# tkkiran/Robust-Conditional-GAN

Hardware: AMD Instinct MI355X
Metric: images/sec G+D train step (CIFAR-10 RCGAN bs=64) (higher is better)
Workload: dtype bf16

## Files before the change

### include/rcgan_hip.h

```cpp
#ifndef RCGAN_HIP_H
#define RCGAN_HIP_H

#include <stddef.h>
#include <stdint.h>

#ifdef __cplusplus
extern "C" {
#endif

#define RCGAN_OK 0
#define RCGAN_EINVALID_ARG (-1)
#define RCGAN_EUNSUPPORTED_SHAPE (-2)
#define RCGAN_EWORKSPACE_TOO_SMALL (-3)
#define RCGAN_EHIP (-4)
#define RCGAN_ERCCL (-5)

#define RCGAN_F32 0
#define RCGAN_BF16 1
#define RCGAN_F16 2

#define RCGAN_ACT_NONE 0
#define RCGAN_ACT_RELU 1
#define RCGAN_ACT_LRELU 2
#define RCGAN_ACT_TANH 3
// ... 285 lines not shown
int rcgan_poly3_rowsum(rcgan_ctx* ctx, int nq, int nr, int d, int n_seg, const float* q, const int32_t* q_off, const float* r,
                       const int32_t* r_off, double gamma, double coef0, int exclude_same_row, double* rowsum);

int rcgan_adam_tf(rcgan_ctx* ctx, size_t count, float* w, const float* g, float* m, float* v,
                  const float* hyper, float beta1, float beta2, float eps, float clip, float grad_scale);
int rcgan_adam_tf_host(rcgan_ctx* ctx, size_t count, float* w, const float* g, float* m, float* v,
                       float lr, float t, float beta1, float beta2, float eps, float clip, float grad_scale);
int rcgan_fill_f32(rcgan_ctx* ctx, size_t count, float* p, float value);
int rcgan_copy_words(rcgan_ctx* ctx, size_t count, const void* src, void* dst);

int rcgan_conv_stats_ok(const rcgan_conv_desc* d);
size_t rcgan_conv_stats_bytes(const rcgan_conv_desc* d);
int rcgan_conv2d_fwd_stats(rcgan_ctx* ctx, const rcgan_conv_desc* d, const void* x, const void* prepared, const float* bias,
                           const void* residual, void* y, float* tile_sums);
int rcgan_bn_stats_from_tiles(rcgan_ctx* ctx, const rcgan_conv_desc* d, int nseg, float eps, const float* tile_sums, float* mean, float* rstd);
int rcgan_bn_apply_segments(rcgan_ctx* ctx, int nseg, int n_per_seg, int rows_per_sample, int c, int n_labels, int dtype, const void* x,
                            const int32_t* labels, const float* gamma, const float* beta, const float* mean, const float* rstd, int act,
                            void* y, void* ws, size_t ws_bytes);

int rcgan_set_grad_scale(rcgan_ctx* ctx, float host_scale, const float* dev_scale);

#define RCGAN_F32_PRECISION_HIGHEST 0
#define RCGAN_F32_PRECISION_HIGH 1
int rcgan_set_f32_matmul_precision(rcgan_ctx* ctx, int precision);
int rcgan_grad_finite_check(rcgan_ctx* ctx, size_t count, const float* g, float* ls_state);
int rcgan_adam_tf_dyn(rcgan_ctx* ctx, size_t count, float* w, const float* g, float* m, float* v, float lr, const float* t_dev,
                      float beta1, float beta2, float eps, float clip, float grad_scale, const float* ls_state);
int rcgan_loss_scale_update(rcgan_ctx* ctx, float* ls_state, float* t_dev0, float* t_dev1, float growth_interval, float min_scale,
                            float max_scale);

// ... 26 lines not shown
```

### robust-conditional-gan_amd/_lib.py

```python
import ctypes as C
import os

_HERE = os.path.dirname(os.path.abspath(__file__))
LIB_PATH = os.environ.get("RCGAN_LIB_PATH") or os.path.join(_HERE, "librcgan_hip.so")
LIB_PATH_F16 = os.environ.get("RCGAN_LIB_PATH_F16") or os.path.join(_HERE, "librcgan_hip_f16.so")

F32, BF16, F16 = 0, 1, 2
ACT_NONE, ACT_RELU, ACT_LRELU, ACT_TANH, ACT_SIGMOID = 0, 1, 2, 3, 4
CONV_IN_UPSAMPLE2X, CONV_IN_RELU, CONV_ACCUMULATE, CONV_FORCE_DIRECT, CONV_OUT_MEANPOOL2, CONV_RESID_UPSAMPLE2X = 1, 2, 4, 8, 16, 32
LOSS_HINGE_REAL, LOSS_HINGE_FAKE, LOSS_NEG_MEAN, LOSS_CE_ONES, LOSS_CE_ZEROS = 0, 1, 2, 3, 4
QUERY_TR_READ = 0
AUG_COLOR, AUG_TRANSLATION, AUG_CUTOUT = 1, 2, 4
AUG_POLICIES = {"color": AUG_COLOR, "translation": AUG_TRANSLATION, "cutout": AUG_CUTOUT}
F32_PRECISION_HIGHEST, F32_PRECISION_HIGH = 0, 1
F32_PRECISIONS = {"highest": F32_PRECISION_HIGHEST, "high": F32_PRECISION_HIGH}

RCGAN_EHIP, RCGAN_ERCCL = -4, -5
EINVALID_ARG, EUNSUPPORTED_SHAPE, EWORKSPACE_TOO_SMALL = -1, -2, -3
ERRORS = {-1: "RCGAN_EINVALID_ARG", -2: "RCGAN_EUNSUPPORTED_SHAPE", -3: "RCGAN_EWORKSPACE_TOO_SMALL",
          -4: "RCGAN_EHIP", -5: "RCGAN_ERCCL"}


def source_hash():
    import glob
# ... 195 lines not shown
    "rcgan_class_moments_bytes": (SZ, [I, I]),
    "rcgan_class_moments_accum": (I, [P, I, I, I, P, P, P]),
    "rcgan_knn_radius": (I, [P, I, I, I, I, P, P, P]),
    "rcgan_ball_query": (I, [P, I, I, I, I, P, P, P, P, P, P, P]),
    "rcgan_poly3_rowsum": (I, [P, I, I, I, I, P, P, P, P, C.c_double, C.c_double, I, P]),
    "rcgan_sgd_momentum": (I, [P, SZ, SZ, P, P, P, P, F, F, I, F]),
    "rcgan_augment_cifar": (I, [P, I, I, P, P, P, P, I, I, P, P]),
    "rcgan_adam_tf": (I, [P, SZ, P, P, P, P, P, F, F, F, F, F]),
    "rcgan_adam_tf_host": (I, [P, SZ, P, P, P, P, F, F, F, F, F, F, F]),
    "rcgan_fill_f32": (I, [P, SZ, P, F]),
    "rcgan_copy_words": (I, [P, SZ, P, P]),
    "rcgan_conv_stats_ok": (I, [DP]),
    "rcgan_conv_stats_bytes": (SZ, [DP]),
    "rcgan_conv2d_fwd_stats": (I, [P, DP, P, P, P, P, P, P]),
    "rcgan_bn_stats_from_tiles": (I, [P, DP, I, F, P, P, P]),
    "rcgan_bn_apply_segments": (I, [P, I, I, I, I, I, I, P, P, P, P, P, P, I, P, P, SZ]),
    "rcgan_comm_unique_id": (I, [P]),
    "rcgan_comm_init": (I, [P, P, I, I]),
    "rcgan_comm_init_stub": (I, [P, I]),
    "rcgan_comm_destroy": (I, [P]),
    "rcgan_comm_world": (I, [P]),
    "rcgan_allreduce_sum": (I, [P, P, SZ]),
    "rcgan_allreduce_sum_buckets": (I, [P, I, P, P]),
    "rcgan_allreduce_sum_async": (I, [P, P, SZ]),
    "rcgan_allreduce_join": (I, [P]),
    "rcgan_comm_count": (I, [P, P]),
    "rcgan_allreduce_bf16_scratch_bytes": (SZ, [I, P]),
    "rcgan_allreduce_sum_bf16_buckets": (I, [P, I, P, P, P, SZ]),
    "rcgan_comm_stub_model": (I, [P, C.c_double, C.c_double]),
    "rcgan_comm_load_error": (C.c_char_p, []),
# ... 33 lines not shown
```

### robust-conditional-gan_amd/csrc/api.hip

```cpp
#include "conv_wgrad.h"
#include "small_gemm.h"
#include "step_inputs.h"
#include "conv_image.h"


size_t direct_wgrad_ws_bytes(const rcgan_conv_desc* d);
template <typename T> int direct_fwd(rcgan_ctx*, const rcgan_conv_desc*, const T*, const float*, const float*, const float*, T*, int n_cols = 0);
template <typename T> int direct_dgrad(rcgan_ctx*, const rcgan_conv_desc*, const T*, const float*, const float*, const float*, const T*, T*, int);
template <typename T> int direct_wgrad(rcgan_ctx*, const rcgan_conv_desc*, const T*, const T*, float*, float*, int, void*, size_t);
template <typename T> int direct_wgrad_cols(rcgan_ctx*, const rcgan_conv_desc*, const T*, const T*, int, const float*, float*, int, void*, size_t);
size_t direct_wgrad_cols_ws_bytes(const rcgan_conv_desc* d, int c1);
template <typename T> int colsum_launch(rcgan_ctx*, const T*, long, int, float*, int, float*);
template <typename T> int linear_fwd(rcgan_ctx*, long, long, long, const T*, const float*, const float*, const float*, T*);
template <typename T> int linear_dgrad(rcgan_ctx*, long, long, long, const T*, const float*, const float*, T*, int);
template <typename T> int linear_wgrad(rcgan_ctx*, long, long, long, const T*, const T*, float*, float*, int, void*, size_t);
size_t linear_wgrad_ws_bytes(long m, long k, long n);
template <typename T> int sumpool2_masked_launch(rcgan_ctx*, int, int, int, int, const T*, const T*, T*, int);
int small_fwd_kind(const rcgan_conv_desc* d);
int small_dgrad_kind(const rcgan_conv_desc* d);
int small_wgrad_kind(const rcgan_conv_desc* d);
size_t small_wgrad_ws_bytes(const rcgan_conv_desc* d);
template <typename T> int small_fwd(rcgan_ctx*, const rcgan_conv_desc*, int, const T*, const float*, const float*, T*);
template <typename T> int small_dgrad(rcgan_ctx*, const rcgan_conv_desc*, int, const T*, const float*, T*, int);
template <typename T> int small_wgrad(rcgan_ctx*, const rcgan_conv_desc*, int, const T*, const T*, float*, float*, int, void*, size_t);
// ... 566 lines not shown
      a.PT = d->kh - 1 - a.PT; a.PL = d->kw - 1 - a.PL;
      if (up) a.accumulate = 0;
    }
  }
  return RCGAN_OK;
}

int rcgan_conv2d_fwd(rcgan_ctx* ctx, const rcgan_conv_desc* d, const void* x, const void* prepared, const float* bias, void* y) {
  return rcgan_conv2d_fwd_residual(ctx, d, x, prepared, bias, nullptr, y);
}

int rcgan_conv_stats_ok(const rcgan_conv_desc* d) {
  if (!d || !mfma_eligible(d) || d->stride != 1 || d->cout != 256) return 0;
  if (d->flags & (RCGAN_CONV_OUT_MEANPOOL2 | RCGAN_CONV_ACCUMULATE | RCGAN_CONV_IN_RELU | RCGAN_CONV_FORCE_DIRECT)) return 0;
  if (((long)d->n * d->h * d->w) % 256 != 0) return 0;
  if ((d->flags & RCGAN_CONV_RESID_UPSAMPLE2X) && !rcgan_conv_resid_up_ok(d)) return 0;
  MfmaConvArgs a;
  if (mfma_conv_pose(nullptr, d, CONV_FWD, nullptr, nullptr, nullptr, false, nullptr, &a)) return 0;
  if (a.up && !(mfma_phase_filters(d) && mfma_conv8_phase_form(a))) return 0;
  return mfma_conv_is_p8(a) ? 1 : 0;
}

size_t rcgan_conv_stats_bytes(const rcgan_conv_desc* d) {
  return d ? (size_t)((long)d->n * d->h * d->w / 256) * d->cout * 2 * sizeof(float) : 0;
}

int rcgan_conv2d_fwd_stats(rcgan_ctx* ctx, const rcgan_conv_desc* d, const void* x, const void* prepared, const float* bias,
                           const void* residual, void* y, float* tile_sums) {
  int rc = check_desc(ctx, d);
  if (rc) return rc;
// ... 55 lines not shown
  int rc = check_desc(ctx, d);
  if (rc) return rc;
  RC_REQUIRE(ctx, x && prepared && y && mean && rstd && gamma && beta, "null argument");
  RC_REQUIRE(ctx, segments >= 1 && d->n % segments == 0, "segments must divide the batch");
  if (!rcgan_conv_bn_in_ok(d)) RC_FAIL(ctx, RCGAN_EUNSUPPORTED_SHAPE, "no kernel applies a batch norm to this convolution's staged input (rcgan_conv_bn_in_ok)");
  if (residual == nullptr && img_fwd_bn_ok(d)) return img_fwd_bn(ctx, d, x, prepared, bias, y, mean, rstd, gamma, beta, labels, segments, act);
  RC_REQUIRE(ctx, mfma_bn_in_route(d), "residual form needs a halo-patch kernel");
  MfmaConvArgs a;
  rc = mfma_conv_pose(ctx, d, CONV_FWD, x, prepared, bias, residual != nullptr, y, &a);
  if (rc) return rc;
  rc = ensure_selftest(ctx);
  if (rc) return rc;
  a.resid = (const bf16_t*)residual;
  a.bn_mean = mean; a.bn_rstd = rstd; a.bn_gamma = gamma; a.bn_beta = beta; a.bn_labels = labels;
  a.bn_seg_samples = d->n / segments; a.bn_act = act;
  return mfma_conv_launch(ctx, a);
}

int rcgan_conv2d_fwd_residual(rcgan_ctx* ctx, const rcgan_conv_desc* d, const void* x, const void* prepared, const float* bias,
                              const void* residual, void* y) {
  int rc = check_desc(ctx, d);
  if (rc) return rc;
  if (residual != nullptr && !mfma_eligible(d)) {
    RC_REQUIRE(ctx, !(d->flags & RCGAN_CONV_RESID_UPSAMPLE2X), "half-resolution residual not available for this convolution (rcgan_conv_resid_up_ok)");
    RC_REQUIRE(ctx, residual != y, "residual must not alias the output");
    rc = rcgan_conv2d_fwd_residual(ctx, d, x, prepared, bias, nullptr, y);
    if (rc) return rc;
    int oh, ow, p;
    same_pad(d->h, d->kh, d->stride, &oh, &p);
    same_pad(d->w, d->kw, d->stride, &ow, &p);
// ... 230 lines not shown
```

### robust-conditional-gan_amd/csrc/bn.hip

```cpp
#include "common.h"
#include "conv_mfma.h"
#include "bn_plan.h"

template <typename T, int MODE>
__global__ __launch_bounds__(256) void bn_partial_kernel(long rows, int c, long rows_per_group, const T* x, const T* y,
                                                         const T* dy, const float* mean, const float* rstd, int act,
                                                         float* partial) {
  __shared__ float red[2][4][64];
  const int col = blockIdx.x * 64 + (threadIdx.x & 63);
  const int rl = threadIdx.x >> 6;
  const long rb = (long)blockIdx.y * rows_per_group;
  long re = rb + rows_per_group;
  if (re > rows) re = rows;
  float s1 = 0.f, s2 = 0.f;
  if (col < c) {
    float mu = 0.f, rs = 1.f;
    if (MODE == 1) { mu = mean[col]; rs = rstd[col]; }
    for (long r = rb + rl; r < re; r += 4) {
      const long off = r * c + col;
      if (MODE == 0) {
        float v = Elem<T>::ld(x + off);
        s1 += v; s2 += v * v;
      } else {
        float g = Elem<T>::ld(dy + off);
// ... 786 lines not shown
    float o[8];
#pragma unroll
    for (int j = 0; j < 8; ++j) o[j] = rs[j] * gm[j] * gv[j] + p[j] * xv[j] + q[j];
    if (accumulate_dx) {
      float d[8];
      ld8(dx + off, d);
#pragma unroll
      for (int j = 0; j < 8; ++j) o[j] += d[j];
    }
    st8(dx + off, o);
  }
}

__global__ __launch_bounds__(256) void bn_tile_stats_finish_kernel(const float* __restrict__ part, int c, int tps, int ngroups, long group_stride,
                                                                   double inv_count, float eps, float* mean, float* rstd) {
  __shared__ double red[2][16][16];
  const int cl = threadIdx.x & 15, sub = threadIdx.x >> 4, ch = blockIdx.x * 16 + cl, sg = blockIdx.y;
  double s1 = 0.0, s2 = 0.0;
  for (int g = 0; g < ngroups; ++g) {
    const long t0 = (long)g * group_stride + (long)sg * tps;
    for (int tb = sub; tb < tps; tb += 16 * 8) {
      float2 v[8];
#pragma unroll
      for (int q = 0; q < 8; ++q) {
        const int t = tb + q * 16;
        v[q] = t < tps ? *(const float2*)(part + ((t0 + t) * c + ch) * 2) : make_float2(0.f, 0.f);
      }
#pragma unroll
      for (int q = 0; q < 8; ++q) { s1 += (double)v[q].x; s2 += (double)v[q].y; }
    }
  }
  red[0][sub][cl] = s1; red[1][sub][cl] = s2;
  __syncthreads();
  if (sub == 0) {
    double a1 = 0.0, a2 = 0.0;
#pragma unroll
    for (int q = 0; q < 16; ++q) { a1 += red[0][q][cl]; a2 += red[1][q][cl]; }
    const double mu = a1 * inv_count;
    double var = a2 * inv_count - mu * mu;
    if (var < 0.0) var = 0.0;
    mean[(long)sg * c + ch] = (float)mu;
    rstd[(long)sg * c + ch] = (float)(1.0 / sqrt(var + (double)eps));
  }
}

int bn_tile_stats_finish_launch(rcgan_ctx* ctx, const float* part, int c, int nseg, int tiles_per_seg, int ngroups, long group_stride,
                                double count, float eps, float* mean, float* rstd) {
  RC_REQUIRE(ctx, c % 16 == 0 && tiles_per_seg >= 1, "bad tile statistics layout");
  hipLaunchKernelGGL(bn_tile_stats_finish_kernel, dim3(c / 16, nseg), dim3(256), 0, ctx->stream, part, c, tiles_per_seg, ngroups, group_stride,
                     1.0 / count, eps, mean, rstd);
  RC_LAUNCH_CHECK(ctx);
  return RCGAN_OK;
}


template <typename T>
__global__ __launch_bounds__(256) void bn_sample_partial_kernel(int rows_per_sample, int c, const T* x, const T* y, const T* dy,
// ... 399 lines not shown
```

### robust-conditional-gan_amd/csrc/conv_mfma.hip

```cpp
#include <vector>
#include "conv_mfma.h"
#include "small_gemm.h"
#include "step_inputs.h"
#include "mfma_util.h"

#define LDS_PITCH 72

template <int BM, int BN>
__global__ __launch_bounds__(256) void conv_mfma_kernel(MfmaConvArgs a) {
  extern __shared__ __attribute__((aligned(16))) unsigned char smem[];
  bf16_t* As = (bf16_t*)smem;
  bf16_t* Bs = As + 2 * BM * LDS_PITCH;
  constexpr int AR = BM / 32, BR = BN / 32;
  constexpr int TM = BM / 2, TN = BN / 2;
  constexpr int NI = TN / 16, NJ = TM / 16;

  const int tid = threadIdx.x, lane = tid & 63, wave = tid >> 6;
  const int wm = wave & 1, wn = wave >> 1;
  const long m0 = (long)blockIdx.x * BM;
  const int co0 = blockIdx.y * BN;
  const int chunk = tid & 7, lrow = tid >> 3;
  const int K = a.KH * a.KW * a.Cin;
  const int KT = K / 64;
  const int Hs = a.up ? (a.H >> 1) : a.H, Ws = a.up ? (a.W >> 1) : a.W;
// ... 941 lines not shown
static ConvRoute mfma_conv_route(const MfmaConvArgs& a) {
  static const int p8_min = env_int("RCGAN_P8_MINBLK", 200);
  static const int p8n_min = env_int("RCGAN_P8N_MINBLK", 190);
  static const int ks2_max = env_int("RCGAN_KS2_MAXBLK", 576);
  static const int halo = env_int("RCGAN_P8_HALO", 1), halo_n = env_int("RCGAN_P8N_HALO", 1);
  static const int t128_min = env_int("RCGAN_T128_MINBLK", 384);
  static const int t256_min = env_int("RCGAN_T256_MINBLK", 1 << 30);
  if (a.phase == MFMA_FORM_PHASE || a.phase == MFMA_FORM_GATHER) {
    const bool whole = a.phase == MFMA_FORM_PHASE ? ((a.M >> 2) % 256 == 0) : (a.M % 256 == 0);
    const long b8 = (a.M / 256) * (a.Cout / 256), b8n = (a.M / 256) * (a.Cout / 128);
    if (a.phase == MFMA_FORM_GATHER) {
      const int gather_min = env_int("RCGAN_H8N_GATHER_MINBLK", 190);
      if (halo_n && whole && a.Cout % 128 == 0 && b8n >= gather_min && mfma_conv8n_halo_takes(a)) return CR_H8N;
    }
    if (whole && a.Cout % 256 == 0 && b8 >= p8_min && 4 * b8 >= 3 * (long)cdiv(b8, 256) * 256)
      return (halo && !a.stats && mfma_conv8_halo_takes(a)) ? CR_H8 : CR_P8;
    if (whole && a.Cout % 128 == 0 && b8n >= p8n_min)
      return (a.phase == MFMA_FORM_PHASE && halo_n && mfma_conv8n_halo_takes(a)) ? CR_H8N : CR_P8N;
    return (a.M / 64) * (a.Cout / 64) <= ks2_max ? CR_PHASE_KS2 : CR_PHASE;
  }
  MfmaConvArgs b = a;
  b.phase = mfma_conv8_phase_form(a) ? MFMA_FORM_PHASE : MFMA_FORM_PLAIN;
  const bool off32 = (long)a.N * a.H * a.W * a.Cin < (1L << 32);
  const long b8 = (long)cdiv(a.M, 256) * (a.Cout / 256), b8n = (long)cdiv(a.M, 256) * (a.Cout / 128);
  const bool fit8 = 4 * b8 >= 3 * (long)cdiv(b8, 256) * 256;
  if (a.Cout % 256 == 0 && a.zero != nullptr && off32 && b8 >= p8_min && fit8) return (halo && !a.stats && mfma_conv8_halo_takes(b)) ? CR_H8 : CR_P8;
  if (a.Cout % 128 == 0 && a.zero != nullptr && b8n >= p8n_min) return (halo_n && mfma_conv8n_halo_takes(b)) ? CR_H8N : CR_P8N;
  if (a.Cout % 256 == 0 && b8 >= t256_min && a.zero != nullptr) return CR_T256;
  if (a.Cout % 128 == 0 && b8n >= t256_min && a.zero != nullptr) return CR_T256N;
  if (a.Cout % 128 == 0 && (long)cdiv(a.M, 128) * (a.Cout / 128) >= t128_min) return CR_T128;
  return CR_64;
}

bool mfma_conv_is_p8(const MfmaConvArgs& a) {
  if (a.phase != MFMA_FORM_PLAIN || a.Cin % 64 || a.Cout % 64) return false;
  const ConvRoute r = mfma_conv_route(a);
  return r == CR_H8 || r == CR_P8;
}

int mfma_conv_bn_route(const MfmaConvArgs& a) {
  if (a.phase != MFMA_FORM_PLAIN || a.Cin % 64 || a.Cout % 64 || a.zero == nullptr || a.stats || a.relu_in || a.Cin > 1024) return 0;
  const ConvRoute r = mfma_conv_route(a);
  return r == CR_H8 ? 1 : r == CR_H8N ? 2 : 0;
}

int mfma_conv_launch(rcgan_ctx* ctx, const MfmaConvArgs& a_in) {
  MfmaConvArgs a = a_in;
  a.stamps = (unsigned long long*)ctx->dbg_stamps;
  if (a.Cin % 64 || a.Cout % 64) RC_FAIL(ctx, RCGAN_EUNSUPPORTED_SHAPE, "channels %d -> %d", a.Cin, a.Cout);
  const ConvRoute r = mfma_conv_route(a);
  if (a.bn_mean && !(a.phase == MFMA_FORM_PLAIN && !a.stats && !a.relu_in && a.Cin <= 1024 && a.zero != nullptr && (r == CR_H8 || r == CR_H8N)))
    RC_FAIL(ctx, RCGAN_EUNSUPPORTED_SHAPE, "batch norm on the staged input needs a halo-patch kernel (rcgan_conv_bn_in_ok)");
  if (a.stats && !(a.phase == MFMA_FORM_PLAIN && a.zero != nullptr && (r == CR_H8 || r == CR_P8)))
    RC_FAIL(ctx, RCGAN_EUNSUPPORTED_SHAPE, "tile statistics need the 256 x 256 kernel (rcgan_conv_stats_ok)");
  switch (r) {
    case CR_H8: case CR_P8: return mfma_conv8_launch(ctx, a, true, r == CR_H8);
    case CR_H8N: case CR_P8N: return mfma_conv8_launch(ctx, a, false, r == CR_H8N);
    case CR_PHASE_KS2: return a.phase == MFMA_FORM_PHASE ? launch_conv_glds_phase<64, 64, 2, 2, 1>(ctx, a) : launch_conv_glds_phase<64, 64, 2, 2, 2>(ctx, a);
    case CR_PHASE: return a.phase == MFMA_FORM_PHASE ? launch_conv_glds_phase<64, 64, 2, 1, 1>(ctx, a) : launch_conv_glds_phase<64, 64, 2, 1, 2>(ctx, a);
    case CR_T256: return launch_conv_glds<256, 256, 2>(ctx, a);
    case CR_T256N: return launch_conv_glds<256, 128, 2>(ctx, a);
    case CR_T128: return launch_conv_mfma<128, 128>(ctx, a);
    default: return launch_conv_mfma<64, 64>(ctx, a);
  }
}

// ... 60 lines not shown
```

### robust-conditional-gan_amd/csrc/conv_mfma8h.hip

```cpp
#include "conv_mfma.h"
#include "mfma_util.h"

#ifndef H8_ABLATE
#define H8_ABLATE 0
#endif

namespace {

template <int N> __device__ __forceinline__ void wait_vm() {
  if constexpr (N == 0) asm volatile("s_waitcnt vmcnt(0)" ::: "memory");
  else if constexpr (N == 1) asm volatile("s_waitcnt vmcnt(1)" ::: "memory");
  else if constexpr (N == 2) asm volatile("s_waitcnt vmcnt(2)" ::: "memory");
  else if constexpr (N == 3) asm volatile("s_waitcnt vmcnt(3)" ::: "memory");
  else if constexpr (N == 4) asm volatile("s_waitcnt vmcnt(4)" ::: "memory");
  else if constexpr (N == 5) asm volatile("s_waitcnt vmcnt(5)" ::: "memory");
  else if constexpr (N == 6) asm volatile("s_waitcnt vmcnt(6)" ::: "memory");
  else if constexpr (N == 7) asm volatile("s_waitcnt vmcnt(7)" ::: "memory");
  else if constexpr (N == 8) asm volatile("s_waitcnt vmcnt(8)" ::: "memory");
  else if constexpr (N == 9) asm volatile("s_waitcnt vmcnt(9)" ::: "memory");
  else if constexpr (N == 10) asm volatile("s_waitcnt vmcnt(10)" ::: "memory");
  else if constexpr (N == 11) asm volatile("s_waitcnt vmcnt(11)" ::: "memory");
  else if constexpr (N == 12) asm volatile("s_waitcnt vmcnt(12)" ::: "memory");
  else static_assert(N == 0, "unsupported vmcnt immediate");
}
// ... 60 lines not shown
__device__ __forceinline__ H8BnTab h8_bn_tab_load(const float* tab, int cin, int ch0) {
  return H8BnTab{*(const float4*)(tab + ch0), *(const float4*)(tab + ch0 + 4), *(const float4*)(tab + cin + ch0), *(const float4*)(tab + cin + ch0 + 4)};
}
__device__ __forceinline__ uint32_t h8_bn_word(uint32_t w, float ia, float ib, float ca, float cb, float relu_floor, bool keep) {
  float lo = __fmaf_rn(h16_lo(w), ia, ca), hi = __fmaf_rn(h16_hi(w), ib, cb);
  lo = fmaxf(lo, relu_floor); hi = fmaxf(hi, relu_floor);
  return keep ? pack_h16x2(lo, hi) : w;
}
__device__ __forceinline__ void h8_bn_stage(int q, uint4& v, const H8BnTab& t, float relu_floor, bool keep) {
  if (q == 0) v.x = h8_bn_word(v.x, t.i0.x, t.i0.y, t.c0.x, t.c0.y, relu_floor, keep);
  if (q == 1) v.y = h8_bn_word(v.y, t.i0.z, t.i0.w, t.c0.z, t.c0.w, relu_floor, keep);
  if (q == 2) v.z = h8_bn_word(v.z, t.i1.x, t.i1.y, t.c1.x, t.c1.y, relu_floor, keep);
  if (q == 3) v.w = h8_bn_word(v.w, t.i1.z, t.i1.w, t.c1.z, t.c1.w, relu_floor, keep);
}

template <int LW, bool RELU, bool PHM, bool BNIN = false>
__global__ __launch_bounds__(512) void conv_mfma_h8_kernel(MfmaConvArgs a) {
  extern __shared__ __attribute__((aligned(16))) unsigned char smem[];
  constexpr int W = 1 << LW, TR = 256 >> LW;
  constexpr int NT = PHM ? 4 : 9;
  constexpr int NTI = PHM ? (BNIN ? 1 : 2) : 6;
  constexpr int PC = W + H8_PC_EXTRA, PR = TR + 2;
  constexpr int NPX = PR * PC, NROWS = h8_patch_rows(LW), NP = NROWS / 8;
  constexpr int PATCH = NROWS * 128;
  constexpr int WBUF = 2 * H8_HALF;
  constexpr int WOFF = 0, P0OFF = 2 * WBUF, P1OFF = 2 * WBUF + PATCH;
  static_assert(WBUF == 32768, "the filter buffers are toggled with ^ 0x8000");
  constexpr int MAXP = (NP + 7) / 8;
  constexpr int PPT = (MAXP + NTI - 1) / NTI;
  static_assert(MAXP <= 6 && NTI <= NT - 2, "a wavefront issues its patch pieces during the first taps of a chunk");
  static_assert((PR - 1) * PC * 128 + PC * 128 < 65536, "tap offsets are ds_read immediates");
// ... 249 lines not shown
      __builtin_amdgcn_sched_barrier(0);
      raw_barrier();
      const bool bn_here = BNIN && (PHM ? tap == 2 : (tap >= 2 && tap - 2 < NTI));
      if (bn_here) mma_bn(1, 0, PHM ? 0 : tap - 2, PHM ? 2 : tap - 1, c + 1);
      else mma(1, 0);
      raw_barrier();
      wad ^= WBUF;
    }
    const int pdelta = (c & 1) ? -PATCH : PATCH;
#pragma unroll
    for (int sx = 0; sx < 16; ++sx) AD[sx] += pdelta;
  }
  if (!grp) wg_barrier();

  stamp(3);
  conv_epilogue(acc, a.bias, a.mask, a.resid, a.out, a.accumulate, a.M, a.Cout, m0 + wm * 128, co0 + wn * 64, lane,
                RowPhase{PHM ? 1 : 0, PHM ? a.lw - 1 : a.lw, PHM ? a.lh - 1 : a.lh, ph, pw, mbase}, a.resid_up ? a.lw : -1, a.lh);
  if (a.stamps) {
    stamp(4);
    wait_vm<0>();
    stamp(5);
  }
}

namespace {
constexpr int H8N_WTILE = 128 * 128;
constexpr int h8n_lds_bytes(int lw) { return 2 * h8_patch_rows(lw) * 128 + 4 * H8N_WTILE; }
}

template <int LW, bool RELU, bool PHM, bool BNIN = false, int NPASS = 1, bool GATHER = false>
__global__ __launch_bounds__(512) void conv_mfma_h8n_kernel(MfmaConvArgs a) {
  static_assert(NPASS == 1 || (NPASS == 2 && PHM && !BNIN), "two passes: the sub-pixel form without a batch norm on the patch");
// ... 254 lines not shown
    const long mbase = PHM ? (long)(tph0 + pp) * Mph : 0;
    conv_epilogue(acc, a.bias, a.mask, a.resid, a.out, a.accumulate, a.M, a.Cout, mbase + ms0 + wm * 64, co0 + wn * 64, lane,
                  RowPhase{PHM ? 1 : 0, PHM ? a.lw - 1 : a.lw, PHM ? a.lh - 1 : a.lh, ph, pw, mbase}, a.resid_up ? a.lw : -1, a.lh);
  }
  if (next_pass) {
#pragma unroll
    for (int i = 0; i < 4; ++i)
#pragma unroll
      for (int j = 0; j < 4; ++j) acc[i][j] = (f32x4_t){0.f, 0.f, 0.f, 0.f};
    if (grp) wg_barrier();
  }
  }
}

bool mfma_conv8_halo_takes(const MfmaConvArgs& a) {
  if (a.KH != 3 || a.KW != 3 || a.stats || a.lw < 0 || a.lh < 0 || a.M % 256 || a.Cin % 64 || a.Cout % 256) return false;
  if ((long)a.N * a.H * a.W * a.Cin >= (1L << 31) || (long)a.Cout * 9 * a.Cin >= (1L << 31)) return false;
  if (a.phase == 0) return a.PT == 1 && a.PL == 1 && !a.up && (a.lw == 4 || a.lw == 5) && (a.H << a.lw) % 256 == 0;
  if (a.phase == 1) return a.up && a.wph != nullptr && (a.lw == 5 || a.lw == 6) && a.lh >= 1 && ((a.H >> 1) << (a.lw - 1)) % 256 == 0 && (a.M >> 2) % 256 == 0;
  return false;
}

#define H8_BN_MAX_CIN 1024
template <int LW, bool RELU, bool PHM, bool BNIN = false>
static int launch8h(rcgan_ctx* ctx, const MfmaConvArgs& a) {
  static bool attr_set = false;
  const size_t lds = h8_lds_bytes(LW) + (BNIN ? 2 * H8_BN_MAX_CIN * sizeof(float) : 0);
  if (!attr_set) {
    RC_HIP(ctx, hipFuncSetAttribute((const void*)conv_mfma_h8_kernel<LW, RELU, PHM, BNIN>, hipFuncAttributeMaxDynamicSharedMemorySize, (int)lds));
    attr_set = true;
  }
  dim3 grid(cdiv(a.M, 256), a.Cout / 256);
  {
    ProfScope ps(ctx, RCGAN_PROF_CONV_P8, 2.0 * (double)a.M * 9 * a.Cin * a.Cout, 2.0 * (double)a.M * (PHM ? 4 : 9) * a.Cin * a.Cout);
    if (BNIN && ps.on) ctx->prof_bn_in++;
    hipLaunchKernelGGL((conv_mfma_h8_kernel<LW, RELU, PHM, BNIN>), grid, dim3(512), lds, ctx->stream, a);
  }
  RC_LAUNCH_CHECK(ctx);
  return RCGAN_OK;
}

int mfma_conv8_halo_launch(rcgan_ctx* ctx, const MfmaConvArgs& a) {
  MfmaConvArgs b = a;
  b.stamps = (unsigned long long*)ctx->dbg_stamps;
  if (a.bn_mean) {
    if (a.relu_in || a.Cin > H8_BN_MAX_CIN || (a.bn_act != RCGAN_ACT_NONE && a.bn_act != RCGAN_ACT_RELU))
      RC_FAIL(ctx, RCGAN_EUNSUPPORTED_SHAPE, "batch norm on the staged patch: no input ReLU, Cin <= %d, activation none / ReLU", H8_BN_MAX_CIN);
    if (a.phase == 1) return a.lw == 6 ? launch8h<5, false, true, true>(ctx, b) : launch8h<4, false, true, true>(ctx, b);
    return a.lw == 5 ? launch8h<5, false, false, true>(ctx, b) : launch8h<4, false, false, true>(ctx, b);
  }
  if (a.phase == 1) {
    if (a.lw == 6) return a.relu_in ? launch8h<5, true, true>(ctx, b) : launch8h<5, false, true>(ctx, b);
    return a.relu_in ? launch8h<4, true, true>(ctx, b) : launch8h<4, false, true>(ctx, b);
  }
  if (a.lw == 5) return a.relu_in ? launch8h<5, true, false>(ctx, b) : launch8h<5, false, false>(ctx, b);
  return a.relu_in ? launch8h<4, true, false>(ctx, b) : launch8h<4, false, false>(ctx, b);
}

bool mfma_conv8n_halo_takes(const MfmaConvArgs& a) {
  if (a.KH != 3 || a.KW != 3 || a.stats || a.lw < 0 || a.lh < 0 || a.M % 256 || a.Cin % 64 || a.Cout % 128) return false;
  if ((long)a.N * a.H * a.W * a.Cin >= (1L << 31) || (long)a.Cout * 16 * a.Cin >= (1L << 31)) return false;
  if (a.phase == 2) return !a.up && a.wph != nullptr && !a.bn_mean && (a.lw == 5 || a.lw == 6) && a.lh >= 1 && ((a.H >> 1) << (a.lw - 1)) % 256 == 0 &&
                           ((a.Cin >> 6) & ((a.Cin >> 6) - 1)) == 0;
  if (a.phase == 0) return a.PT == 1 && a.PL == 1 && !a.up && (a.lw == 4 || a.lw == 5) && (a.H << a.lw) % 256 == 0;
// ... 48 lines not shown
```

### robust-conditional-gan_amd/ops.py

```python
import ctypes as C
import os

import torch

from . import _lib as L
from .runtime import DT


def _p(t):
    return C.c_void_p(t.ptr) if t is not None else None


def same_pad(n, k, s):
    out = -(-n // s)
    tot = max((out - 1) * s + k - n, 0)
    return out, tot // 2


def zeros_like_grad(ctx, t):
    g = ctx.empty(t.shape, t.dtype)
    ctx.check(ctx.lib.rcgan_fill_f32(ctx.h, (g.nbytes + 3) // 4, g.ptr, 0.0))
    return g


# ... 216 lines not shown
                ranges = None
        if ranges is not None:
            ra = (C.c_size_t * max(len(ranges), 1))(*ranges)
            opt = L.SnAdam(grp.value.data_ptr(), grp.grad.data_ptr(), grp.m.data_ptr(), grp.v.data_ptr(), grp.count, grp.hyper.data_ptr(),
                           fa["beta1"], fa["beta2"], fa.get("eps", 1e-8), fa.get("clip", 0.0), fa["grad_scale"], len(ranges) // 2, ra)
            ctx.check(ctx.lib.rcgan_sn_bwd_adam(ctx.h, bi, len(todo), C.byref(opt)))
            fa["done"] = True
            return
        ctx.check(ctx.lib.rcgan_sn_bwd(ctx.h, bi, len(todo)))
    if any(p.req for p, _, _ in entries):
        ctx.record(bw)
        ctx.sn_partial.append(bw)
    return weights


FUSE_BN_STATS = os.environ.get("RCGAN_FUSE_BN_STATS", "0") == "1"


def conv2d(ctx, x, weight, bias, k, stride=1, in_up=False, in_relu=False, accumulate_into=None, force_direct=False,
           residual=None, residual_up=False, want_stats=False):
    if isinstance(x, BnPending):
        pend = x
        n, hs, ws_, cin = pend.shape
        cout = weight.param.shape[-1]
        assert weight.param.shape == (k, k, cin, cout), (weight.param.shape, (k, k, cin, cout))
        bh, bw = (hs * 2, ws_ * 2) if in_up else (hs, ws_)
        bflags = (L.CONV_IN_UPSAMPLE2X if in_up else 0) | (L.CONV_RESID_UPSAMPLE2X if (residual is not None and residual_up) else 0)
        bdesc = L.ConvDesc(n, bh, bw, cin, cout, k, k, stride, pend.dtype, bflags)
        if (not in_relu and accumulate_into is None and not force_direct and not ctx.recording and stride == 1
                and pend.act in (L.ACT_NONE, L.ACT_RELU) and ctx.lib.rcgan_conv_bn_in_ok(C.byref(bdesc))
                and (residual is None or (residual.shape == ((n, bh // 2, bw // 2, cout) if residual_up else (n, bh, bw, cout))
                                          and (not residual_up or ctx.lib.rcgan_conv_resid_up_ok(C.byref(bdesc)))))):
            y = ctx.empty((n, bh, bw, cout), pend.dtype)
            pdesc = L.ConvDesc(n, bh, bw, cin, cout, k, k, stride, pend.dtype, L.CONV_IN_UPSAMPLE2X if in_up else 0)
            rc = ctx.lib.rcgan_conv2d_fwd_bn_residual(ctx.h, C.byref(bdesc), _p(pend.x), _p(weight.prepared(pdesc)), _p(bias), _p(residual), _p(y),
                                                      pend.segments, _p(pend.labels), _p(pend.gamma), _p(pend.beta), _p(pend.mean),
                                                      _p(pend.rstd), pend.act)
            if rc == 0:
                return y
            if rc != L.EUNSUPPORTED_SHAPE:
                ctx.check(rc)
        x = pend.materialize()
    n, hs, ws_, cin = x.shape
    h, w = (hs * 2, ws_ * 2) if in_up else (hs, ws_)
    cout = weight.param.shape[-1]
    assert weight.param.shape == (k, k, cin, cout), (weight.param.shape, (k, k, cin, cout))
    flags = (L.CONV_IN_UPSAMPLE2X if in_up else 0) | (L.CONV_IN_RELU if in_relu else 0) | (L.CONV_FORCE_DIRECT if force_direct else 0)
    oh, _ = same_pad(h, k, stride)
    ow, _ = same_pad(w, k, stride)
    desc = L.ConvDesc(n, h, w, cin, cout, k, k, stride, x.dtype, flags)
    prep = weight.prepared(desc)
    if accumulate_into is not None:
        y = accumulate_into
        assert y.shape == (n, oh, ow, cout)
        fdesc = L.ConvDesc(n, h, w, cin, cout, k, k, stride, x.dtype, flags | L.CONV_ACCUMULATE)
    else:
        y = ctx.empty((n, oh, ow, cout), x.dtype)
        fdesc = desc
    use_rf = (RF_CONV and weight.rf_frag is not None and residual is None and not in_up and not force_direct
              and bool(ctx.lib.rcgan_conv_rf_ok(C.byref(fdesc))))
    sdesc = None
    if want_stats and FUSE_BN_STATS and accumulate_into is None and not in_relu and x.dtype != L.F32:
        sd = L.ConvDesc(n, h, w, cin, cout, k, k, stride, x.dtype, flags | (L.CONV_RESID_UPSAMPLE2X if (residual is not None and residual_up) else 0))
        if ctx.lib.rcgan_conv_stats_ok(C.byref(sd)):
            sdesc = sd
    if sdesc is not None:
        assert residual is None or residual.shape == ((n, oh // 2, ow // 2, cout) if residual_up else (n, oh, ow, cout))
        sums = ctx.empty((ctx.lib.rcgan_conv_stats_bytes(C.byref(sdesc)) // 4,), L.F32)
        ctx.check(ctx.lib.rcgan_conv2d_fwd_stats(ctx.h, C.byref(sdesc), _p(x), _p(prep), _p(bias), _p(residual), _p(y), _p(sums)))
        y.tile_stats = (sdesc, sums)
    elif residual is not None and residual_up:
        assert residual.shape == (n, oh // 2, ow // 2, cout) and accumulate_into is None, (residual.shape, (n, oh, ow, cout))
        rdesc = L.ConvDesc(n, h, w, cin, cout, k, k, stride, x.dtype, flags | L.CONV_RESID_UPSAMPLE2X)
        if ctx.lib.rcgan_conv_resid_up_ok(C.byref(rdesc)):
            ctx.check(ctx.lib.rcgan_conv2d_fwd_residual(ctx.h, C.byref(rdesc), _p(x), _p(prep), _p(bias), _p(residual), _p(y)))
        else:
            up = ctx.empty((n, oh, ow, cout), x.dtype)
# ... 270 lines not shown
            ctx.check(ctx.lib.rcgan_bn_apply_fwd(ctx.h, n, rps, c, self.n_labels, x.dtype, _p(x), _p(self.labels), _p(self.gamma), _p(self.beta),
                                                 _p(self.mean), _p(self.rstd), self.act, _p(y), C.c_void_p(ctx.ws_ptr), ctx.ws_bytes))
        return y


BN_INTO_CONV = os.environ.get("RCGAN_BN_INTO_CONV", "1") != "0"


def batch_norm_act(ctx, x, gamma, beta, act=L.ACT_NONE, labels=None, n_labels=1, moving=None, decay=0.9, eps=1e-5, segments=1,
                   defer_apply=False, stats_out=None):
    n, rps, c = _rows(x)
    if stats_out is not None and (segments > 1 or defer_apply):
        raise NotImplementedError("stats_out is for the plain batch norm (one segment, applied at once)")
    rows = n * rps
    tile = getattr(x, "tile_stats", None) if moving is None else None
    if (defer_apply and BN_INTO_CONV and not ctx.recording and moving is None and tile is None and x.dtype != L.F32
            and n % max(segments, 1) == 0):
        mean = ctx.empty((max(segments, 1), c), L.F32)
        rstd = ctx.empty((max(segments, 1), c), L.F32)
        if segments > 1:
            ctx.check(ctx.lib.rcgan_bn_fwd_segments(ctx.h, segments, n // segments, rps, c, n_labels, x.dtype, _p(x), _p(labels), _p(gamma),
                                                    _p(beta), eps, act, _p(mean), _p(rstd), None, C.c_void_p(ctx.ws_ptr), ctx.ws_bytes))
        else:
            ctx.check(ctx.lib.rcgan_bn_stats(ctx.h, rows, c, x.dtype, _p(x), eps, _p(mean), _p(rstd), None, None, decay,
                                             C.c_void_p(ctx.ws_ptr), ctx.ws_bytes))
        return BnPending(ctx, x, gamma, beta, labels, n_labels, mean, rstd, act, max(segments, 1))
    if segments > 1 and labels is None and n % segments == 0 and ((ctx.recording and (x.req or gamma.req or beta.req)) or moving is not None):
        ns = n // segments
        y = ctx.empty(x.shape, x.dtype)
        mm, mv = moving if moving is not None else (None, None)
        stats = []
        for sg in range(segments):
            xs, ys = x.rows(sg * ns, (sg + 1) * ns), y.rows(sg * ns, (sg + 1) * ns)
            mean, rstd = ctx.empty((c,), L.F32), ctx.empty((c,), L.F32)
            ctx.check(ctx.lib.rcgan_bn_stats(ctx.h, ns * rps, c, x.dtype, _p(xs), eps, _p(mean), _p(rstd), _p(mm), _p(mv), decay,
# ... 525 lines not shown
```

Baseline: 61890.

## Fuse batch-norm tile statistics into halo conv epilogue and enable by default

Result: no change. 62330, median of 6 (+0.7%).

```diff
diff --git a/include/rcgan_hip.h b/include/rcgan_hip.h
--- a/include/rcgan_hip.h
+++ b/include/rcgan_hip.h
@@ -323,6 +323,10 @@
 int rcgan_conv2d_fwd_stats(rcgan_ctx* ctx, const rcgan_conv_desc* d, const void* x, const void* prepared, const float* bias,
                            const void* residual, void* y, float* tile_sums);
 int rcgan_bn_stats_from_tiles(rcgan_ctx* ctx, const rcgan_conv_desc* d, int nseg, float eps, const float* tile_sums, float* mean, float* rstd);
+int rcgan_conv_bn_stats_ok(const rcgan_conv_desc* d);
+int rcgan_conv2d_fwd_bn_stats(rcgan_ctx* ctx, const rcgan_conv_desc* d, const void* x, const void* prepared, const float* bias,
+                              const void* residual , void* y, int segments, const int32_t* labels, const float* gamma,
+                              const float* beta, const float* mean, const float* rstd, int act, float* tile_sums);
 int rcgan_bn_apply_segments(rcgan_ctx* ctx, int nseg, int n_per_seg, int rows_per_sample, int c, int n_labels, int dtype, const void* x,
                             const int32_t* labels, const float* gamma, const float* beta, const float* mean, const float* rstd, int act,
                             void* y, void* ws, size_t ws_bytes);
diff --git a/robust-conditional-gan_amd/_lib.py b/robust-conditional-gan_amd/_lib.py
--- a/robust-conditional-gan_amd/_lib.py
+++ b/robust-conditional-gan_amd/_lib.py
@@ -233,6 +233,8 @@
     "rcgan_conv_stats_bytes": (SZ, [DP]),
     "rcgan_conv2d_fwd_stats": (I, [P, DP, P, P, P, P, P, P]),
     "rcgan_bn_stats_from_tiles": (I, [P, DP, I, F, P, P, P]),
+    "rcgan_conv_bn_stats_ok": (I, [DP]),
+    "rcgan_conv2d_fwd_bn_stats": (I, [P, DP, P, P, P, P, P, I, P, P, P, P, P, I, P]),
     "rcgan_bn_apply_segments": (I, [P, I, I, I, I, I, I, P, P, P, P, P, P, I, P, P, SZ]),
     "rcgan_comm_unique_id": (I, [P]),
     "rcgan_comm_init": (I, [P, P, I, I]),
diff --git a/robust-conditional-gan_amd/csrc/api.hip b/robust-conditional-gan_amd/csrc/api.hip
--- a/robust-conditional-gan_amd/csrc/api.hip
+++ b/robust-conditional-gan_amd/csrc/api.hip
@@ -604,6 +604,8 @@
   if (!d || !mfma_eligible(d) || d->stride != 1 || d->cout != 256) return 0;
   if (d->flags & (RCGAN_CONV_OUT_MEANPOOL2 | RCGAN_CONV_ACCUMULATE | RCGAN_CONV_IN_RELU | RCGAN_CONV_FORCE_DIRECT)) return 0;
   if (((long)d->n * d->h * d->w) % 256 != 0) return 0;
+  const long px = (long)d->h * d->w;
+  if ((d->flags & RCGAN_CONV_IN_UPSAMPLE2X) ? (px / 4) % 256 != 0 : (px % 256 != 0 && 256 % px != 0)) return 0;
   if ((d->flags & RCGAN_CONV_RESID_UPSAMPLE2X) && !rcgan_conv_resid_up_ok(d)) return 0;
   MfmaConvArgs a;
   if (mfma_conv_pose(nullptr, d, CONV_FWD, nullptr, nullptr, nullptr, false, nullptr, &a)) return 0;
@@ -689,6 +691,32 @@
   a.resid = (const bf16_t*)residual;
   a.bn_mean = mean; a.bn_rstd = rstd; a.bn_gamma = gamma; a.bn_beta = beta; a.bn_labels = labels;
   a.bn_seg_samples = d->n / segments; a.bn_act = act;
+  return mfma_conv_launch(ctx, a);
+}
+
+int rcgan_conv_bn_stats_ok(const rcgan_conv_desc* d) {
+  return (d && d->dtype == RCGAN_H16 && rcgan_conv_stats_ok(d) && mfma_bn_in_route(d) == 1) ? 1 : 0;
+}
+
+int rcgan_conv2d_fwd_bn_stats(rcgan_ctx* ctx, const rcgan_conv_desc* d, const void* x, const void* prepared, const float* bias, const void* residual,
+                              void* y, int segments, const int32_t* labels, const float* gamma, const float* beta, const float* mean,
+                              const float* rstd, int act, float* tile_sums) {
+  if (!ctx) return RCGAN_EINVALID_ARG;
+  int rc = check_desc(ctx, d);
+  if (rc) return rc;
+  RC_REQUIRE(ctx, x && prepared && y && mean && rstd && gamma && beta && tile_sums, "null argument");
+  RC_REQUIRE(ctx, segments >= 1 && d->n % segments == 0, "segments must divide the batch");
+  if (!rcgan_conv_bn_stats_ok(d))
+    RC_FAIL(ctx, RCGAN_EUNSUPPORTED_SHAPE, "no kernel takes a batch norm on this convolution's input and leaves tile statistics (rcgan_conv_bn_stats_ok)");
+  MfmaConvArgs a;
+  rc = mfma_conv_pose(ctx, d, CONV_FWD, x, prepared, bias, residual != nullptr, y, &a);
+  if (rc) return rc;
+  rc = ensure_selftest(ctx);
+  if (rc) return rc;
+  a.resid = (const bf16_t*)residual;
+  a.bn_mean = mean; a.bn_rstd = rstd; a.bn_gamma = gamma; a.bn_beta = beta; a.bn_labels = labels;
+  a.bn_seg_samples = d->n / segments; a.bn_act = act;
+  a.stats = tile_sums;
   return mfma_conv_launch(ctx, a);
 }
 
diff --git a/robust-conditional-gan_amd/csrc/bn.hip b/robust-conditional-gan_amd/csrc/bn.hip
--- a/robust-conditional-gan_amd/csrc/bn.hip
+++ b/robust-conditional-gan_amd/csrc/bn.hip
@@ -824,33 +824,34 @@
 
 __global__ __launch_bounds__(256) void bn_tile_stats_finish_kernel(const float* __restrict__ part, int c, int tps, int ngroups, long group_stride,
                                                                    double inv_count, float eps, float* mean, float* rstd) {
-  __shared__ double red[2][16][16];
-  const int cl = threadIdx.x & 15, sub = threadIdx.x >> 4, ch = blockIdx.x * 16 + cl, sg = blockIdx.y;
-  double s1 = 0.0, s2 = 0.0;
-  for (int g = 0; g < ngroups; ++g) {
-    const long t0 = (long)g * group_stride + (long)sg * tps;
-    for (int tb = sub; tb < tps; tb += 16 * 8) {
-      float2 v[8];
-#pragma unroll
-      for (int q = 0; q < 8; ++q) {
-        const int t = tb + q * 16;
-        v[q] = t < tps ? *(const float2*)(part + ((t0 + t) * c + ch) * 2) : make_float2(0.f, 0.f);
-      }
-#pragma unroll
-      for (int q = 0; q < 8; ++q) { s1 += (double)v[q].x; s2 += (double)v[q].y; }
-    }
-  }
-  red[0][sub][cl] = s1; red[1][sub][cl] = s2;
+  __shared__ double red[32][8][4];
+  const int cp = threadIdx.x & 7, sub = threadIdx.x >> 3, ch = blockIdx.x * 16 + cp * 2, sg = blockIdx.y;
+  const int ntiles = ngroups * tps;
+  double s[4] = {0.0, 0.0, 0.0, 0.0};
+  for (int tb = sub; tb < ntiles; tb += 32 * 16) {
+    float4 v[16];
+#pragma unroll
+    for (int q = 0; q < 16; ++q) {
+      const int idx = tb + q * 32;
+      const int g = idx / tps, t = idx - g * tps;
+      v[q] = idx < ntiles ? *(const float4*)(part + (((long)g * group_stride + (long)sg * tps + t) * c + ch) * 2) : make_float4(0.f, 0.f, 0.f, 0.f);
+    }
+#pragma unroll
+    for (int q = 0; q < 16; ++q) { s[0] += (double)v[q].x; s[1] += (double)v[q].y; s[2] += (double)v[q].z; s[3] += (double)v[q].w; }
+  }
+#pragma unroll
+  for (int k = 0; k < 4; ++k) red[sub][cp][k] = s[k];
   __syncthreads();
-  if (sub == 0) {
+  if (threadIdx.x < 16) {
+    const int cl = threadIdx.x;
     double a1 = 0.0, a2 = 0.0;
 #pragma unroll
-    for (int q = 0; q < 16; ++q) { a1 += red[0][q][cl]; a2 += red[1][q][cl]; }
+    for (int q = 0; q < 32; ++q) { a1 += red[q][cl >> 1][(cl & 1) * 2]; a2 += red[q][cl >> 1][(cl & 1) * 2 + 1]; }
     const double mu = a1 * inv_count;
     double var = a2 * inv_count - mu * mu;
     if (var < 0.0) var = 0.0;
-    mean[(long)sg * c + ch] = (float)mu;
-    rstd[(long)sg * c + ch] = (float)(1.0 / sqrt(var + (double)eps));
+    mean[(long)sg * c + blockIdx.x * 16 + cl] = (float)mu;
+    rstd[(long)sg * c + blockIdx.x * 16 + cl] = (float)(1.0 / sqrt(var + (double)eps));
   }
 }
 
diff --git a/robust-conditional-gan_amd/csrc/conv_mfma.hip b/robust-conditional-gan_amd/csrc/conv_mfma.hip
--- a/robust-conditional-gan_amd/csrc/conv_mfma.hip
+++ b/robust-conditional-gan_amd/csrc/conv_mfma.hip
@@ -979,7 +979,7 @@
       if (halo_n && whole && a.Cout % 128 == 0 && b8n >= gather_min && mfma_conv8n_halo_takes(a)) return CR_H8N;
     }
     if (whole && a.Cout % 256 == 0 && b8 >= p8_min && 4 * b8 >= 3 * (long)cdiv(b8, 256) * 256)
-      return (halo && !a.stats && mfma_conv8_halo_takes(a)) ? CR_H8 : CR_P8;
+      return (halo && mfma_conv8_halo_takes(a)) ? CR_H8 : CR_P8;
     if (whole && a.Cout % 128 == 0 && b8n >= p8n_min)
       return (a.phase == MFMA_FORM_PHASE && halo_n && mfma_conv8n_halo_takes(a)) ? CR_H8N : CR_P8N;
     return (a.M / 64) * (a.Cout / 64) <= ks2_max ? CR_PHASE_KS2 : CR_PHASE;
@@ -989,7 +989,7 @@
   const bool off32 = (long)a.N * a.H * a.W * a.Cin < (1L << 32);
   const long b8 = (long)cdiv(a.M, 256) * (a.Cout / 256), b8n = (long)cdiv(a.M, 256) * (a.Cout / 128);
   const bool fit8 = 4 * b8 >= 3 * (long)cdiv(b8, 256) * 256;
-  if (a.Cout % 256 == 0 && a.zero != nullptr && off32 && b8 >= p8_min && fit8) return (halo && !a.stats && mfma_conv8_halo_takes(b)) ? CR_H8 : CR_P8;
+  if (a.Cout % 256 == 0 && a.zero != nullptr && off32 && b8 >= p8_min && fit8) return (halo && mfma_conv8_halo_takes(b)) ? CR_H8 : CR_P8;
   if (a.Cout % 128 == 0 && a.zero != nullptr && b8n >= p8n_min) return (halo_n && mfma_conv8n_halo_takes(b)) ? CR_H8N : CR_P8N;
   if (a.Cout % 256 == 0 && b8 >= t256_min && a.zero != nullptr) return CR_T256;
   if (a.Cout % 128 == 0 && b8n >= t256_min && a.zero != nullptr) return CR_T256N;
@@ -1004,9 +1004,9 @@
 }
 
 int mfma_conv_bn_route(const MfmaConvArgs& a) {
-  if (a.phase != MFMA_FORM_PLAIN || a.Cin % 64 || a.Cout % 64 || a.zero == nullptr || a.stats || a.relu_in || a.Cin > 1024) return 0;
+  if (a.phase != MFMA_FORM_PLAIN || a.Cin % 64 || a.Cout % 64 || a.zero == nullptr || a.relu_in || a.Cin > 1024) return 0;
   const ConvRoute r = mfma_conv_route(a);
-  return r == CR_H8 ? 1 : r == CR_H8N ? 2 : 0;
+  return r == CR_H8 ? 1 : (r == CR_H8N && !a.stats) ? 2 : 0;
 }
 
 int mfma_conv_launch(rcgan_ctx* ctx, const MfmaConvArgs& a_in) {
@@ -1014,7 +1014,7 @@
   a.stamps = (unsigned long long*)ctx->dbg_stamps;
   if (a.Cin % 64 || a.Cout % 64) RC_FAIL(ctx, RCGAN_EUNSUPPORTED_SHAPE, "channels %d -> %d", a.Cin, a.Cout);
   const ConvRoute r = mfma_conv_route(a);
-  if (a.bn_mean && !(a.phase == MFMA_FORM_PLAIN && !a.stats && !a.relu_in && a.Cin <= 1024 && a.zero != nullptr && (r == CR_H8 || r == CR_H8N)))
+  if (a.bn_mean && !(a.phase == MFMA_FORM_PLAIN && !a.relu_in && a.Cin <= 1024 && a.zero != nullptr && (r == CR_H8 || r == CR_H8N)))
     RC_FAIL(ctx, RCGAN_EUNSUPPORTED_SHAPE, "batch norm on the staged input needs a halo-patch kernel (rcgan_conv_bn_in_ok)");
   if (a.stats && !(a.phase == MFMA_FORM_PLAIN && a.zero != nullptr && (r == CR_H8 || r == CR_P8)))
     RC_FAIL(ctx, RCGAN_EUNSUPPORTED_SHAPE, "tile statistics need the 256 x 256 kernel (rcgan_conv_stats_ok)");
diff --git a/robust-conditional-gan_amd/csrc/conv_mfma8h.hip b/robust-conditional-gan_amd/csrc/conv_mfma8h.hip
--- a/robust-conditional-gan_amd/csrc/conv_mfma8h.hip
+++ b/robust-conditional-gan_amd/csrc/conv_mfma8h.hip
@@ -98,7 +98,7 @@
   if (q == 3) v.w = h8_bn_word(v.w, t.i1.z, t.i1.w, t.c1.z, t.c1.w, relu_floor, keep);
 }
 
-template <int LW, bool RELU, bool PHM, bool BNIN = false>
+template <int LW, bool RELU, bool PHM, bool BNIN = false, bool STATS = false>
 __global__ __launch_bounds__(512) void conv_mfma_h8_kernel(MfmaConvArgs a) {
   extern __shared__ __attribute__((aligned(16))) unsigned char smem[];
   constexpr int W = 1 << LW, TR = 256 >> LW;
@@ -378,8 +378,35 @@
   if (!grp) wg_barrier();
 
   stamp(3);
-  conv_epilogue(acc, a.bias, a.mask, a.resid, a.out, a.accumulate, a.M, a.Cout, m0 + wm * 128, co0 + wn * 64, lane,
-                RowPhase{PHM ? 1 : 0, PHM ? a.lw - 1 : a.lw, PHM ? a.lh - 1 : a.lh, ph, pw, mbase}, a.resid_up ? a.lw : -1, a.lh);
+  if constexpr (STATS) {
+    float st[2][16];
+#pragma unroll
+    for (int p = 0; p < 2; ++p)
+#pragma unroll
+      for (int k = 0; k < 16; ++k) st[p][k] = 0.f;
+    conv_epilogue<4, 8, RowPhase, true>(acc, a.bias, nullptr, a.resid, a.out, 0, a.M, a.Cout, m0 + wm * 128, co0 + wn * 64, lane,
+                                        RowPhase{PHM ? 1 : 0, PHM ? a.lw - 1 : a.lw, PHM ? a.lh - 1 : a.lh, ph, pw, mbase}, a.resid_up ? a.lw : -1, a.lh, st);
+#pragma unroll
+    for (int p = 0; p < 2; ++p)
+#pragma unroll
+      for (int k = 0; k < 16; ++k) st[p][k] = row16_sum(st[p][k]);
+    float* const red = (float*)smem;
+    if ((lane & 15) == 0) {
+      const int row = lane >> 4;
+#pragma unroll
+      for (int p = 0; p < 2; ++p)
+#pragma unroll
+        for (int e = 0; e < 8; ++e) {
+          const int ch = wn * 64 + (2 * p + (row & 1)) * 16 + (row >> 1) * 8 + e;
+          *(float2*)(red + (wm * 256 + ch) * 2) = make_float2(st[p][e], st[p][8 + e]);
+        }
+    }
+    __syncthreads();
+    a.stats[((long)mt * a.Cout + co0) * 2 + tid] = red[tid] + red[512 + tid];
+  } else {
+    conv_epilogue(acc, a.bias, a.mask, a.resid, a.out, a.accumulate, a.M, a.Cout, m0 + wm * 128, co0 + wn * 64, lane,
+                  RowPhase{PHM ? 1 : 0, PHM ? a.lw - 1 : a.lw, PHM ? a.lh - 1 : a.lh, ph, pw, mbase}, a.resid_up ? a.lw : -1, a.lh);
+  }
   if (a.stamps) {
     stamp(4);
     wait_vm<0>();
@@ -664,7 +691,8 @@
 }
 
 bool mfma_conv8_halo_takes(const MfmaConvArgs& a) {
-  if (a.KH != 3 || a.KW != 3 || a.stats || a.lw < 0 || a.lh < 0 || a.M % 256 || a.Cin % 64 || a.Cout % 256) return false;
+  if (a.stats && (a.relu_in || a.accumulate || a.mask)) return false;
+  if (a.KH != 3 || a.KW != 3 || a.lw < 0 || a.lh < 0 || a.M % 256 || a.Cin % 64 || a.Cout % 256) return false;
   if ((long)a.N * a.H * a.W * a.Cin >= (1L << 31) || (long)a.Cout * 9 * a.Cin >= (1L << 31)) return false;
   if (a.phase == 0) return a.PT == 1 && a.PL == 1 && !a.up && (a.lw == 4 || a.lw == 5) && (a.H << a.lw) % 256 == 0;
   if (a.phase == 1) return a.up && a.wph != nullptr && (a.lw == 5 || a.lw == 6) && a.lh >= 1 && ((a.H >> 1) << (a.lw - 1)) % 256 == 0 && (a.M >> 2) % 256 == 0;
@@ -672,19 +700,19 @@
 }
 
 #define H8_BN_MAX_CIN 1024
-template <int LW, bool RELU, bool PHM, bool BNIN = false>
+template <int LW, bool RELU, bool PHM, bool BNIN = false, bool STATS = false>
 static int launch8h(rcgan_ctx* ctx, const MfmaConvArgs& a) {
   static bool attr_set = false;
   const size_t lds = h8_lds_bytes(LW) + (BNIN ? 2 * H8_BN_MAX_CIN * sizeof(float) : 0);
   if (!attr_set) {
-    RC_HIP(ctx, hipFuncSetAttribute((const void*)conv_mfma_h8_kernel<LW, RELU, PHM, BNIN>, hipFuncAttributeMaxDynamicSharedMemorySize, (int)lds));
+    RC_HIP(ctx, hipFuncSetAttribute((const void*)conv_mfma_h8_kernel<LW, RELU, PHM, BNIN, STATS>, hipFuncAttributeMaxDynamicSharedMemorySize, (int)lds));
     attr_set = true;
   }
   dim3 grid(cdiv(a.M, 256), a.Cout / 256);
   {
     ProfScope ps(ctx, RCGAN_PROF_CONV_P8, 2.0 * (double)a.M * 9 * a.Cin * a.Cout, 2.0 * (double)a.M * (PHM ? 4 : 9) * a.Cin * a.Cout);
     if (BNIN && ps.on) ctx->prof_bn_in++;
-    hipLaunchKernelGGL((conv_mfma_h8_kernel<LW, RELU, PHM, BNIN>), grid, dim3(512), lds, ctx->stream, a);
+    hipLaunchKernelGGL((conv_mfma_h8_kernel<LW, RELU, PHM, BNIN, STATS>), grid, dim3(512), lds, ctx->stream, a);
   }
   RC_LAUNCH_CHECK(ctx);
   return RCGAN_OK;
@@ -693,11 +721,20 @@
 int mfma_conv8_halo_launch(rcgan_ctx* ctx, const MfmaConvArgs& a) {
   MfmaConvArgs b = a;
   b.stamps = (unsigned long long*)ctx->dbg_stamps;
+  if (a.stats && (a.relu_in || a.accumulate || a.mask)) RC_FAIL(ctx, RCGAN_EUNSUPPORTED_SHAPE, "tile statistics: unsupported form");
   if (a.bn_mean) {
     if (a.relu_in || a.Cin > H8_BN_MAX_CIN || (a.bn_act != RCGAN_ACT_NONE && a.bn_act != RCGAN_ACT_RELU))
       RC_FAIL(ctx, RCGAN_EUNSUPPORTED_SHAPE, "batch norm on the staged patch: no input ReLU, Cin <= %d, activation none / ReLU", H8_BN_MAX_CIN);
+    if (a.stats) {
+      if (a.phase == 1) return a.lw == 6 ? launch8h<5, false, true, true, true>(ctx, b) : launch8h<4, false, true, true, true>(ctx, b);
+      return a.lw == 5 ? launch8h<5, false, false, true, true>(ctx, b) : launch8h<4, false, false, true, true>(ctx, b);
+    }
     if (a.phase == 1) return a.lw == 6 ? launch8h<5, false, true, true>(ctx, b) : launch8h<4, false, true, true>(ctx, b);
     return a.lw == 5 ? launch8h<5, false, false, true>(ctx, b) : launch8h<4, false, false, true>(ctx, b);
+  }
+  if (a.stats) {
+    if (a.phase == 1) return a.lw == 6 ? launch8h<5, false, true, false, true>(ctx, b) : launch8h<4, false, true, false, true>(ctx, b);
+    return a.lw == 5 ? launch8h<5, false, false, false, true>(ctx, b) : launch8h<4, false, false, false, true>(ctx, b);
   }
   if (a.phase == 1) {
     if (a.lw == 6) return a.relu_in ? launch8h<5, true, true>(ctx, b) : launch8h<5, false, true>(ctx, b);
diff --git a/robust-conditional-gan_amd/ops.py b/robust-conditional-gan_amd/ops.py
--- a/robust-conditional-gan_amd/ops.py
+++ b/robust-conditional-gan_amd/ops.py
@@ -254,7 +254,17 @@
     return weights
 
 
-FUSE_BN_STATS = os.environ.get("RCGAN_FUSE_BN_STATS", "0") == "1"
+def _fuse_bn_stats_setting():
+    v = os.environ.get("RCGAN_FUSE_BN_STATS", FUSE_BN_STATS_DEFAULT)
+    return {"0": 0, "1": 1, "fwd": 2}.get(v, 0)
+
+
+FUSE_BN_STATS_DEFAULT = "fwd"
+FUSE_BN_STATS = _fuse_bn_stats_setting()
+
+
+def _fuse_stats_here(ctx):
+    return FUSE_BN_STATS == 1 or (FUSE_BN_STATS == 2 and not ctx.recording)
 
 
 def conv2d(ctx, x, weight, bias, k, stride=1, in_up=False, in_relu=False, accumulate_into=None, force_direct=False,
@@ -273,6 +283,16 @@
                                           and (not residual_up or ctx.lib.rcgan_conv_resid_up_ok(C.byref(bdesc)))))):
             y = ctx.empty((n, bh, bw, cout), pend.dtype)
             pdesc = L.ConvDesc(n, bh, bw, cin, cout, k, k, stride, pend.dtype, L.CONV_IN_UPSAMPLE2X if in_up else 0)
+            if want_stats and _fuse_stats_here(ctx) and ctx.lib.rcgan_conv_bn_stats_ok(C.byref(bdesc)):
+                sums = ctx.empty((ctx.lib.rcgan_conv_stats_bytes(C.byref(bdesc)) // 4,), L.F32)
+                rc = ctx.lib.rcgan_conv2d_fwd_bn_stats(ctx.h, C.byref(bdesc), _p(pend.x), _p(weight.prepared(pdesc)), _p(bias), _p(residual), _p(y),
+                                                       pend.segments, _p(pend.labels), _p(pend.gamma), _p(pend.beta), _p(pend.mean),
+                                                       _p(pend.rstd), pend.act, _p(sums))
+                if rc == 0:
+                    y.tile_stats = (bdesc, sums)
+                    return y
+                if rc != L.EUNSUPPORTED_SHAPE:
+                    ctx.check(rc)
             rc = ctx.lib.rcgan_conv2d_fwd_bn_residual(ctx.h, C.byref(bdesc), _p(pend.x), _p(weight.prepared(pdesc)), _p(bias), _p(residual), _p(y),
                                                       pend.segments, _p(pend.labels), _p(pend.gamma), _p(pend.beta), _p(pend.mean),
                                                       _p(pend.rstd), pend.act)
@@ -300,7 +320,7 @@
     use_rf = (RF_CONV and weight.rf_frag is not None and residual is None and not in_up and not force_direct
               and bool(ctx.lib.rcgan_conv_rf_ok(C.byref(fdesc))))
     sdesc = None
-    if want_stats and FUSE_BN_STATS and accumulate_into is None and not in_relu and x.dtype != L.F32:
+    if want_stats and _fuse_stats_here(ctx) and accumulate_into is None and not in_relu and x.dtype != L.F32:
         sd = L.ConvDesc(n, h, w, cin, cout, k, k, stride, x.dtype, flags | (L.CONV_RESID_UPSAMPLE2X if (residual is not None and residual_up) else 0))
         if ctx.lib.rcgan_conv_stats_ok(C.byref(sd)):
             sdesc = sd
@@ -601,11 +621,15 @@
         raise NotImplementedError("stats_out is for the plain batch norm (one segment, applied at once)")
     rows = n * rps
     tile = getattr(x, "tile_stats", None) if moving is None else None
-    if (defer_apply and BN_INTO_CONV and not ctx.recording and moving is None and tile is None and x.dtype != L.F32
+    if tile is not None and (n % max(segments, 1) or ((n // max(segments, 1)) * rps) % 256):
+        tile = None
+    if (defer_apply and BN_INTO_CONV and not ctx.recording and moving is None and x.dtype != L.F32
             and n % max(segments, 1) == 0):
         mean = ctx.empty((max(segments, 1), c), L.F32)
         rstd = ctx.empty((max(segments, 1), c), L.F32)
-        if segments > 1:
+        if tile is not None:
+            ctx.check(ctx.lib.rcgan_bn_stats_from_tiles(ctx.h, C.byref(tile[0]), max(segments, 1), eps, _p(tile[1]), _p(mean), _p(rstd)))
+        elif segments > 1:
             ctx.check(ctx.lib.rcgan_bn_fwd_segments(ctx.h, segments, n // segments, rps, c, n_labels, x.dtype, _p(x), _p(labels), _p(gamma),
                                                     _p(beta), eps, act, _p(mean), _p(rstd), None, C.c_void_p(ctx.ws_ptr), ctx.ws_bytes))
         else:
```
